# datawhalechina/torch-rechub

Measured on AMD Instinct MI355X. Metric: CTR train samples/sec, DeepFM Criteo-shape synthetic, higher is better.
Workload: dtype f32

## Files before the change

torch_rechub_amd/csrc/optim.hip:

```cpp
#include "common.h"
#include "wgrad_body.h"

namespace {

constexpr int kMaxTensors = 128;
constexpr int kMaxRing = 1024;
int g_sweep_grid = 0;
int g_deferred_grid = 512;
int g_gate_ns = 32000;
int g_stagger_ns = 15000;

constexpr int kVecPerThread = 4;
constexpr int kChunk4 = RH_BLOCK * kVecPerThread;

struct AdamArgs {
  const int64_t* tdesc;
  const double* hyper;
  int T;
  int zero_grad;
  int64_t total_vblocks;
  int64_t vb_prefix[kMaxTensors + 1];
};

__global__ void adam_prepare_kernel(double* hyper, int64_t* step, float* ring, int64_t ring_mask) {
// ... 17 lines not shown
      ring[2 * (t & ring_mask) + 1] = (float)E;
    }
  }
}

struct AdamScalars {
  float b1, b2, wd, one_m_b1, one_m_b2;
  float c1wd, c2wd2;
  float A, E;
};

static __device__ __forceinline__ void adam_elem(float& p, float g, float& m, float& v, const AdamScalars& h, float A,
                                                 float E) {
  g = fmaf(h.wd, p, g);
  m = fmaf(h.one_m_b1, g - m, m);
  v = fmaf(h.one_m_b2, g * g, v * h.b2);
  p = fmaf(-A, m * __builtin_amdgcn_rcpf(__builtin_amdgcn_sqrtf(v) + E), p);
}
typedef float rh_v2f __attribute__((ext_vector_type(2)));
static __device__ __forceinline__ void adam_pair(rh_v2f& p, rh_v2f g, rh_v2f& m, rh_v2f& v, const AdamScalars& h,
                                                 float A, float E) {
  g = __builtin_elementwise_fma(rh_v2f{h.wd, h.wd}, p, g);
  m = __builtin_elementwise_fma(rh_v2f{h.one_m_b1, h.one_m_b1}, g - m, m);
  v = __builtin_elementwise_fma(rh_v2f{h.one_m_b2, h.one_m_b2}, g * g, v * h.b2);
  rh_v2f d = rh_v2f{__builtin_amdgcn_sqrtf(v.x), __builtin_amdgcn_sqrtf(v.y)} + E;
  d = rh_v2f{__builtin_amdgcn_rcpf(d.x), __builtin_amdgcn_rcpf(d.y)};
  p = __builtin_elementwise_fma(rh_v2f{-A, -A}, m * d, p);
}
static __device__ __forceinline__ void adam_pair_zero_g(rh_v2f& p, rh_v2f& m, rh_v2f& v, const AdamScalars& h, float A,
                                                        float E) {
  m = __builtin_elementwise_fma(rh_v2f{h.c1wd, h.c1wd}, p, m * h.b1);
  v = __builtin_elementwise_fma(rh_v2f{h.c2wd2, h.c2wd2}, p * p, v * h.b2);
  rh_v2f d = rh_v2f{__builtin_amdgcn_sqrtf(v.x), __builtin_amdgcn_sqrtf(v.y)} + E;
  d = rh_v2f{__builtin_amdgcn_rcpf(d.x), __builtin_amdgcn_rcpf(d.y)};
  p = __builtin_elementwise_fma(rh_v2f{-A, -A}, m * d, p);
}
static __device__ __forceinline__ void adam_f4_zero_g(float4& P, float4& M, float4& V, const AdamScalars& h, float A,
                                                      float E) {
  rh_v2f p0{P.x, P.y}, p1{P.z, P.w}, m0{M.x, M.y}, m1{M.z, M.w}, v0{V.x, V.y}, v1{V.z, V.w};
  adam_pair_zero_g(p0, m0, v0, h, A, E);
  adam_pair_zero_g(p1, m1, v1, h, A, E);
  P = make_float4(p0.x, p0.y, p1.x, p1.y);
  M = make_float4(m0.x, m0.y, m1.x, m1.y);
  V = make_float4(v0.x, v0.y, v1.x, v1.y);
}
static __device__ __forceinline__ void adam_f4(float4& P, const float4 G, float4& M, float4& V, const AdamScalars& h,
                                               float A, float E) {
  float4 Pz = P, Mz = M, Vz = V;
  adam_f4_zero_g(Pz, Mz, Vz, h, A, E);
  rh_v2f p0{P.x, P.y}, p1{P.z, P.w}, m0{M.x, M.y}, m1{M.z, M.w}, v0{V.x, V.y}, v1{V.z, V.w};
  adam_pair(p0, rh_v2f{G.x, G.y}, m0, v0, h, A, E);
  adam_pair(p1, rh_v2f{G.z, G.w}, m1, v1, h, A, E);
  P = make_float4(G.x == 0.f ? Pz.x : p0.x, G.y == 0.f ? Pz.y : p0.y, G.z == 0.f ? Pz.z : p1.x, G.w == 0.f ? Pz.w : p1.y);
  M = make_float4(G.x == 0.f ? Mz.x : m0.x, G.y == 0.f ? Mz.y : m0.y, G.z == 0.f ? Mz.z : m1.x, G.w == 0.f ? Mz.w : m1.y);
  V = make_float4(G.x == 0.f ? Vz.x : v0.x, G.y == 0.f ? Vz.y : v0.y, G.z == 0.f ? Vz.z : v1.x, G.w == 0.f ? Vz.w : v1.y);
}
static __device__ __forceinline__ AdamScalars load_scalars(const double* hyper) {
  AdamScalars h;
  h.b1 = (float)hyper[1];
  h.b2 = (float)hyper[2];
  h.wd = (float)hyper[4];
  h.one_m_b1 = (float)hyper[10];
  h.one_m_b2 = (float)hyper[11];
  h.c1wd = h.one_m_b1 * h.wd;
  h.c2wd2 = h.one_m_b2 * h.wd * h.wd;
  h.A = (float)hyper[13];
  h.E = (float)hyper[14];
  return h;
}

__global__ __launch_bounds__(RH_BLOCK) void adam_dense_kernel(const AdamArgs a) {
  const AdamScalars h = load_scalars(a.hyper);
  const int T = a.T;
  for (int64_t vb = blockIdx.x; vb < a.total_vblocks; vb += gridDim.x) {
    int lo = 0, hi = T;
    while (hi - lo > 1) {
      const int mid = (lo + hi) >> 1;
      if (a.vb_prefix[mid] <= vb) lo = mid; else hi = mid;
    }
    const int t = lo;
    float* p = reinterpret_cast<float*>(a.tdesc[0 * T + t]);
    float* g = reinterpret_cast<float*>(a.tdesc[1 * T + t]);
    float* m = reinterpret_cast<float*>(a.tdesc[2 * T + t]);
    float* v = reinterpret_cast<float*>(a.tdesc[3 * T + t]);
    const int64_t n4 = a.tdesc[4 * T + t] / 4;
    const int64_t base4 = (vb - a.vb_prefix[t]) * kChunk4;
    float4 P[kVecPerThread], Gv[kVecPerThread], M[kVecPerThread], V[kVecPerThread];
    bool ok[kVecPerThread];
#pragma unroll
    for (int k = 0; k < kVecPerThread; ++k) {
      const int64_t i4 = base4 + (int64_t)k * RH_BLOCK + threadIdx.x;
      ok[k] = i4 < n4;
      const int64_t j4 = ok[k] ? i4 : 0;
      P[k] = gload<float4>(p + j4 * 4);
      Gv[k] = gload<float4>(g + j4 * 4);
      M[k] = gload<float4>(m + j4 * 4);
      V[k] = gload<float4>(v + j4 * 4);
    }
#pragma unroll
    for (int k = 0; k < kVecPerThread; ++k) {
      if (!ok[k]) continue;
      const int64_t i4 = base4 + (int64_t)k * RH_BLOCK + threadIdx.x;
      const bool gnz = Gv[k].x != 0.f || Gv[k].y != 0.f || Gv[k].z != 0.f || Gv[k].w != 0.f;
      adam_f4(P[k], Gv[k], M[k], V[k], h, h.A, h.E);
      gstore<float4>(p + i4 * 4, P[k]);
      gstore<float4>(m + i4 * 4, M[k]);
      gstore<float4>(v + i4 * 4, V[k]);
      if (a.zero_grad && gnz) gstore<float4>(g + i4 * 4, f4_zero());
    }
  }
}


struct LazyTouchedArgs {
  const int64_t* ldesc;
  const int64_t* field_table;
  const int64_t* idesc;
  const double* hyper;
  const float* ring;
  int ring_mask;
  int T, B, F, spb;
  int* err;
  const int64_t* perm;
  const int64_t* pos;
  int64_t N;
  const int64_t* src_sparse;
  int Fd;
  const float* src_dense;
  int ND;
  const float* src_label;
  int64_t* sparse_out;
  float* dense_out;
  float* label_out;
  int look;
  int look_n;
  int64_t off;
};

struct LazySweepArgs {
  const int64_t* ldesc;
  const double* hyper;
  const float* ring;
  int ring_mask;
  int T;
  int flush;
  int64_t t_value;
  int64_t total_vblocks;
  int64_t vb_prefix[kMaxTensors + 1];
  int touch_blocks, touch_chunks, touch_period;
  int touch_i32;
  LazyTouchedArgs touch;
};

template <int LPR, typename IdxT, bool REFRESH, bool ASSEMBLE = false, bool LOOK = false, bool GRAD = !REFRESH>
static __device__ __forceinline__ void lazy_touched_body(const LazyTouchedArgs& a, int bx, int f);

template <int LPR, bool MERGED>
static __device__ __forceinline__ void lazy_sweep_body(const LazySweepArgs& a, const int bx_, const int gdim_) {
  constexpr int RPB = RH_BLOCK / LPR;
  constexpr int D = 4 * LPR;
  int64_t bid = bx_, nblk = gdim_;
  if (MERGED) {
    const int bx = bx_, P = a.touch_period;
    const int slot_ = bx / P;
    if (bx % P == 0 && slot_ < a.touch_blocks) {
      if (a.touch_i32)
        lazy_touched_body<LPR, int, false>(a.touch, slot_ % a.touch_chunks, slot_ / a.touch_chunks);
      else
        lazy_touched_body<LPR, int64_t, false>(a.touch, slot_ % a.touch_chunks, slot_ / a.touch_chunks);
      return;
    }
    bid = bx - (slot_ + 1 < a.touch_blocks ? slot_ + 1 : a.touch_blocks);
    nblk = (int64_t)gdim_ - a.touch_blocks;
  }
  AdamScalars h = load_scalars(a.hyper);
  const int t = a.t_value >= 0 ? (int)a.t_value : (int)a.hyper[12];
  if (a.t_value >= 0) {
    h.A = a.ring[2 * (t & a.ring_mask)];
    h.E = a.ring[2 * (t & a.ring_mask) + 1];
  }
  const int T = a.T;
  const int q = threadIdx.x % LPR;
  const int slot = threadIdx.x / LPR;
  __shared__ float ring_s[2 * kMaxRing];
  for (int i = threadIdx.x; i < 2 * (a.ring_mask + 1); i += RH_BLOCK) ring_s[i] = a.ring[i];
  __syncthreads();

  struct Unit {
    float *p, *g, *m, *v;
    int* last;
    int64_t r;
    int old;
    bool live, with_g, claimed;
    float4 P, M, V, G;
  };
  auto fetch = [&](int64_t vb, Unit& u) {
    u.live = false;
    if (vb >= a.total_vblocks) return;
    int lo = 0, hi = T;
    while (hi - lo > 1) {
      const int mid = (lo + hi) >> 1;
      if (a.vb_prefix[mid] <= vb) lo = mid; else hi = mid;
    }
    const int ti = lo;
    u.p = reinterpret_cast<float*>(a.ldesc[0 * T + ti]);
    u.g = reinterpret_cast<float*>(a.ldesc[1 * T + ti]);
    u.m = reinterpret_cast<float*>(a.ldesc[2 * T + ti]);
    u.v = reinterpret_cast<float*>(a.ldesc[3 * T + ti]);
    u.last = reinterpret_cast<int*>(a.ldesc[4 * T + ti]);
    const int64_t rows = a.ldesc[5 * T + ti];
    const int64_t K = a.ldesc[6 * T + ti];
    const int64_t w = a.flush ? rows : a.ldesc[7 * T + ti];
    const int64_t wstart = a.flush ? 0 : ((int64_t)(t - 1) % K) * w;
    const int64_t local = (vb - a.vb_prefix[ti]) * RPB + slot;
    u.r = wstart + local;
    if (local >= w || u.r >= rows) return;
    u.with_g = (K == 1);
    const bool claim = MERGED && K != 1;
    u.claimed = claim;
    if (claim) {
      u.old = t;
      if (q == 0) u.old = atomicMax(u.last + u.r, t);
      u.with_g = true;
    } else {
      u.old = gload<int>(u.last + u.r);
    }
    u.P = gload<float4>(u.p + u.r * D + q * 4);
    u.M = gload<float4>(u.m + u.r * D + q * 4);
    u.V = gload<float4>(u.v + u.r * D + q * 4);
    u.G = u.with_g ? gload<float4>(u.g + u.r * D + q * 4) : f4_zero();
    if (claim) u.old = __shfl(u.old, (int)(threadIdx.x % RH_WAVE) - q, RH_WAVE);
    u.live = true;
  };
  auto process = [&](Unit& u) {
    const bool work = u.live && u.old < t;
    const int first = work ? u.old + 1 : t;
    int j = wave_min_uniform(first);
    while (j < t) {
      const int nxt = wave_min_uniform(first > j ? first : t);
      if (first <= j) {
        int jj = j;
        for (; jj + 2 <= nxt; jj += 2) {
          const float2 ae0 = *reinterpret_cast<const float2*>(ring_s + 2 * (jj & a.ring_mask));
          const float2 ae1 = *reinterpret_cast<const float2*>(ring_s + 2 * ((jj + 1) & a.ring_mask));
          __builtin_amdgcn_sched_barrier(0);
          adam_f4_zero_g(u.P, u.M, u.V, h, ae0.x, ae0.y);
          adam_f4_zero_g(u.P, u.M, u.V, h, ae1.x, ae1.y);
        }
        if (jj < nxt) {
          const float2 ae = *reinterpret_cast<const float2*>(ring_s + 2 * (jj & a.ring_mask));
          adam_f4_zero_g(u.P, u.M, u.V, h, ae.x, ae.y);
        }
      }
      j = nxt;
    }
    if (work) {
      if (u.with_g) adam_f4(u.P, u.G, u.M, u.V, h, h.A, h.E);
      else adam_f4_zero_g(u.P, u.M, u.V, h, h.A, h.E);
      gstore<float4>(u.p + u.r * D + q * 4, u.P);
      gstore<float4>(u.m + u.r * D + q * 4, u.M);
      gstore<float4>(u.v + u.r * D + q * 4, u.V);
      if (u.with_g && (u.G.x != 0.f || u.G.y != 0.f || u.G.z != 0.f || u.G.w != 0.f))
        gstore<float4>(u.g + u.r * D + q * 4, f4_zero());
      if (q == 0 && !(MERGED && u.with_g && u.claimed)) u.last[u.r] = t;
    }
  };
  Unit ua, ub;
  fetch(bid, ua);
  for (int64_t vb = bid; vb < a.total_vblocks; vb += 2 * nblk) {
    fetch(vb + nblk, ub);
    process(ua);
    fetch(vb + 2 * nblk, ua);
    process(ub);
  }
}

template <int LPR, bool MERGED = false>
__global__ __launch_bounds__(RH_BLOCK) void adam_lazy_sweep_kernel(const LazySweepArgs a) {
  lazy_sweep_body<LPR, MERGED>(a, (int)blockIdx.x, (int)gridDim.x);
}

template <int LPR, int VPL>
static __device__ __forceinline__ void lazy_sweep_wide_body(const LazySweepArgs& a, const int bx_, const int gdim_) {
  constexpr int RPB = RH_BLOCK / LPR;
  constexpr int D = 4 * LPR * VPL;
  const int64_t bid = bx_, nblk = gdim_;
  AdamScalars h = load_scalars(a.hyper);
  const int t = (int)a.t_value;
  h.A = a.ring[2 * (t & a.ring_mask)];
  h.E = a.ring[2 * (t & a.ring_mask) + 1];
  const int T = a.T;
  const int q = threadIdx.x % LPR;
  const int slot = threadIdx.x / LPR;
  __shared__ float ring_s[2 * kMaxRing];
  for (int i = threadIdx.x; i < 2 * (a.ring_mask + 1); i += RH_BLOCK) ring_s[i] = a.ring[i];
  __syncthreads();
  struct Unit {
    float *p, *m, *v;
    int* last;
    int64_t off;
    int64_t r;
    int old;
    bool live;
    float4 P[VPL], M[VPL], V[VPL];
  };
  auto fetch = [&](int64_t vb, Unit& u) {
    u.live = false;
    if (vb >= a.total_vblocks) return;
    int lo = 0, hi = T;
    while (hi - lo > 1) {
      const int mid = (lo + hi) >> 1;
      if (a.vb_prefix[mid] <= vb) lo = mid; else hi = mid;
    }
    const int ti = lo;
    u.p = reinterpret_cast<float*>(a.ldesc[0 * T + ti]);
    u.m = reinterpret_cast<float*>(a.ldesc[2 * T + ti]);
    u.v = reinterpret_cast<float*>(a.ldesc[3 * T + ti]);
    u.last = reinterpret_cast<int*>(a.ldesc[4 * T + ti]);
    const int64_t rows = a.ldesc[5 * T + ti];
    const int64_t K = a.ldesc[6 * T + ti];
    const int64_t w = a.ldesc[7 * T + ti];
    const int64_t wstart = ((int64_t)(t - 1) % K) * w;
    const int64_t local = (vb - a.vb_prefix[ti]) * RPB + slot;
    u.r = wstart + local;
    if (local >= w || u.r >= rows) return;
    u.off = u.r * D + (int64_t)q * (4 * VPL);
    u.old = gload<int>(u.last + u.r);
#pragma unroll
    for (int k = 0; k < VPL; ++k) {
      u.P[k] = gload<float4>(u.p + u.off + 4 * k);
      u.M[k] = gload<float4>(u.m + u.off + 4 * k);
      u.V[k] = gload<float4>(u.v + u.off + 4 * k);
    }
    u.live = true;
  };
  auto process = [&](Unit& u) {
    const bool work = u.live && u.old < t;
    const int first = work ? u.old + 1 : t;
    int j = wave_min_uniform(first);
    while (j < t) {
      const int nxt = wave_min_uniform(first > j ? first : t);
      if (first <= j) {
        int jj = j;
        for (; jj + 2 <= nxt; jj += 2) {
          const float2 ae0 = *reinterpret_cast<const float2*>(ring_s + 2 * (jj & a.ring_mask));
          const float2 ae1 = *reinterpret_cast<const float2*>(ring_s + 2 * ((jj + 1) & a.ring_mask));
          __builtin_amdgcn_sched_barrier(0);
#pragma unroll
          for (int k = 0; k < VPL; ++k) adam_f4_zero_g(u.P[k], u.M[k], u.V[k], h, ae0.x, ae0.y);
#pragma unroll
          for (int k = 0; k < VPL; ++k) adam_f4_zero_g(u.P[k], u.M[k], u.V[k], h, ae1.x, ae1.y);
        }
        if (jj < nxt) {
          const float2 ae = *reinterpret_cast<const float2*>(ring_s + 2 * (jj & a.ring_mask));
#pragma unroll
          for (int k = 0; k < VPL; ++k) adam_f4_zero_g(u.P[k], u.M[k], u.V[k], h, ae.x, ae.y);
        }
      }
      j = nxt;
    }
    if (work) {
#pragma unroll
      for (int k = 0; k < VPL; ++k) {
        adam_f4_zero_g(u.P[k], u.M[k], u.V[k], h, h.A, h.E);
        gstore<float4>(u.p + u.off + 4 * k, u.P[k]);
        gstore<float4>(u.m + u.off + 4 * k, u.M[k]);
        gstore<float4>(u.v + u.off + 4 * k, u.V[k]);
      }
      if (q == 0) u.last[u.r] = t;
    }
  };
  Unit ua, ub;
  fetch(bid, ua);
  for (int64_t vb = bid; vb < a.total_vblocks; vb += 2 * nblk) {
    fetch(vb + nblk, ub);
    process(ua);
    fetch(vb + 2 * nblk, ua);
    process(ub);
  }
}

template <int LPR, int VPL>
__global__ __launch_bounds__(RH_BLOCK) void adam_lazy_sweep_wide_kernel(const LazySweepArgs a) {
  lazy_sweep_wide_body<LPR, VPL>(a, (int)blockIdx.x, (int)gridDim.x);
}

__global__ void stream_delay_kernel(const long long ticks) {
  const long long t0 = wall_clock64();
  while (wall_clock64() - t0 < ticks) __builtin_amdgcn_s_sleep(16);
}

__global__ void stream_gate_kernel(const long long* gate, const long long expected, const long long ticks, const long long timeout,
                                   int* err, long long* done_host, const long long done_value) {
  if (done_host != nullptr) __hip_atomic_store(done_host, done_value, __ATOMIC_RELAXED, __HIP_MEMORY_SCOPE_SYSTEM);
  const long long t0 = wall_clock64();
  while (__hip_atomic_load(gate, __ATOMIC_ACQUIRE, __HIP_MEMORY_SCOPE_AGENT) - expected < 0) {
    __builtin_amdgcn_s_sleep(8);
    if (wall_clock64() - t0 > timeout) {
      if (err != nullptr) atomicOr(err, RH_ERR_GATE_TIMEOUT);
      return;
    }
  }
  const int slot = 4 + 2 * (int)(expected & 3);
  const long long base = __hip_atomic_load(gate + slot, __ATOMIC_RELAXED, __HIP_MEMORY_SCOPE_AGENT);
  const long long opened = __hip_atomic_load(gate + slot + 1, __ATOMIC_RELAXED, __HIP_MEMORY_SCOPE_AGENT);
  while (__hip_atomic_load(gate + 2, __ATOMIC_RELAXED, __HIP_MEMORY_SCOPE_AGENT) - base < 1 && wall_clock64() - opened < ticks)
    __builtin_amdgcn_s_sleep(4);
}

static __device__ __forceinline__ void gate_open(long long* gate) {
  const long long idx = __hip_atomic_load(gate, __ATOMIC_RELAXED, __HIP_MEMORY_SCOPE_AGENT) + 1;
  const int slot = 4 + 2 * (int)(idx & 3);
  const long long now = (long long)wall_clock64();
  __hip_atomic_store(gate + slot, __hip_atomic_load(gate + 2, __ATOMIC_RELAXED, __HIP_MEMORY_SCOPE_AGENT), __ATOMIC_RELAXED,
                     __HIP_MEMORY_SCOPE_AGENT);
  __hip_atomic_store(gate + slot + 1, now, __ATOMIC_RELAXED, __HIP_MEMORY_SCOPE_AGENT);
  __hip_atomic_store(gate + 1, now, __ATOMIC_RELAXED, __HIP_MEMORY_SCOPE_AGENT);
  __hip_atomic_fetch_add(gate, 1ll, __ATOMIC_RELEASE, __HIP_MEMORY_SCOPE_AGENT);
}

__global__ void stream_gate_open_kernel(long long* gate) { gate_open(gate); }
__global__ void stream_gate_release_kernel(long long* gate) {
  __hip_atomic_fetch_add(gate + 2, 1ll, __ATOMIC_RELAXED, __HIP_MEMORY_SCOPE_AGENT);
}

template <int LPR, typename IdxT, bool REFRESH, bool ASSEMBLE, bool LOOK, bool GRAD>
static __device__ __forceinline__ void lazy_touched_body(const LazyTouchedArgs& a, int bx, int f) {
  constexpr int LPP = RH_BLOCK / LPR;
  constexpr int D = 4 * LPR;
  const int T = a.T, F = a.F;
  const int64_t ti = a.field_table[f];
  if (ti < 0) return;
  const int64_t K = a.ldesc[6 * T + ti];
  if (K == 1) return;
  const int64_t pad = a.field_table[F + f];
  float* p = reinterpret_cast<float*>(a.ldesc[0 * T + ti]);
  float* g = reinterpret_cast<float*>(a.ldesc[1 * T + ti]);
  float* m = reinterpret_cast<float*>(a.ldesc[2 * T + ti]);
  float* v = reinterpret_cast<float*>(a.ldesc[3 * T + ti]);
  int* last = reinterpret_cast<int*>(a.ldesc[4 * T + ti]);
  const int64_t rows = a.ldesc[5 * T + ti];
  const IdxT* ip = reinterpret_cast<const IdxT*>(a.idesc[f]);
  const int64_t st = a.idesc[F + f];
  const int64_t acol = ASSEMBLE ? (reinterpret_cast<const int64_t*>(ip) - a.sparse_out) : 0;
  const int64_t apos = ASSEMBLE ? a.pos[0] : 0;
  const AdamScalars h = load_scalars(a.hyper);
  const int t = (int)a.hyper[12];
  const int q = threadIdx.x % LPR;
  const int slot = threadIdx.x / LPR;
  const int lane = threadIdx.x % RH_WAVE;
  const int64_t nsamp = LOOK ? a.look_n : a.B;
  int64_t b0 = (int64_t)bx * (LOOK ? a.look : a.spb);
  int64_t b1 = (b0 + (LOOK ? a.look : a.spb) < nsamp) ? b0 + (LOOK ? a.look : a.spb) : nsamp;
  __shared__ float ring_t[REFRESH ? 2 * kMaxRing : 2];
  if (REFRESH) {
    for (int i = threadIdx.x; i < 2 * (a.ring_mask + 1); i += RH_BLOCK) ring_t[i] = a.ring[i];
    __syncthreads();
  }
  const float* ring = REFRESH ? ring_t : a.ring;
  const bool pad_pass = !LOOK && REFRESH && pad >= 0 && pad < rows && bx == 0;
  __shared__ int64_t s_look[LOOK ? RH_BLOCK : 1];
  __shared__ int s_nlook;
  const int64_t look_b1 = b1;
  for (int64_t sub = LOOK ? b0 : 0; sub < (LOOK ? look_b1 : 1); sub += RH_BLOCK) {
  if (LOOK) {
    const int64_t w = a.ldesc[7 * T + ti];
    const int64_t ws = ((int64_t)(t - 1) % K) * w;
    if (threadIdx.x == 0) s_nlook = 0;
    __syncthreads();
    const int64_t b = sub + threadIdx.x;
    if (b < look_b1) {
      const int64_t p = (apos + a.off + (int64_t)a.B + b) % a.N;
      const int64_t r = gload<int64_t>(a.src_sparse + gload<int64_t>(a.perm + p) * a.Fd + acol);
      if (r >= ws && r < ws + w && r < rows && r != pad) s_look[atomicAdd(&s_nlook, 1)] = r;
    }
    __syncthreads();
    b0 = 0;
    b1 = s_nlook;
  }
  const int64_t b_end = b1 + (pad_pass ? LPP : 0);
  for (int64_t base = b0; base < b_end; base += LPP) {
    const bool extra = base >= b1;
    const int64_t b = base + slot;
    const bool ok = !extra && b < b1;
    int64_t r;
    if (LOOK) {
      r = s_look[ok ? b : 0];
    } else if (ASSEMBLE) {
      int64_t p = apos + a.off + (ok ? b : b1 - 1);
      if (p >= a.N) p %= a.N;
      if (p < 0) p += a.N;
      r = gload<int64_t>(a.src_sparse + gload<int64_t>(a.perm + p) * a.Fd + acol);
    } else {
      r = (int64_t)gload<IdxT>(ip + (ok ? b : b1 - 1) * st);
    }
    bool valid = ok && (uint64_t)r < (uint64_t)rows && r != pad;
    if (extra) {
      r = pad;
      valid = slot == 0;
    }
    int old = t;
    if (valid && q == 0) {
      old = gload<int>(last + r);
      if (old < t) old = atomicMax(last + r, t);
    }
    old = __shfl(old, lane - q, RH_WAVE);
    bool act = valid && old < t;
    int64_t rr = r;
    if (REFRESH) {
      __shared__ int s_key[LPP];
      __shared__ int s_old[LPP];
      __shared__ int64_t s_row[LPP];
      const int lag = act ? t - old : 0;
      __syncthreads();
      if (q == 0) s_key[slot] = lag;
      __syncthreads();
      int rank = 0;
#pragma unroll 4
      for (int j = 0; j < LPP; ++j) {
        const int kj = s_key[j];
        rank += (kj > lag || (kj == lag && j < slot)) ? 1 : 0;
      }
      constexpr int kPerWave = RH_WAVE / LPR;
      rank = (rank + (bx % (LPP / kPerWave > 0 ? LPP / kPerWave : 1)) * kPerWave) % LPP;
      if (q == 0) {
        s_row[rank] = r;
        s_old[rank] = act ? old : t;
      }
      __syncthreads();
      rr = s_row[slot];
      old = s_old[slot];
      act = old < t;
    }
    float4 P = f4_zero(), M = f4_zero(), V = f4_zero(), G = f4_zero();
    if (act) {
      P = gload<float4>(p + rr * D + q * 4);
      M = gload<float4>(m + rr * D + q * 4);
      V = gload<float4>(v + rr * D + q * 4);
      if (GRAD) G = gload<float4>(g + rr * D + q * 4);
    }
    const int first = act ? old + 1 : t;
    int j = wave_min_uniform(first);
    while (j < t) {
      const int nxt = wave_min_uniform(first > j ? first : t);
      if (first <= j) {
        for (int jj = j; jj < nxt; ++jj) {
          const float A = ring[2 * (jj & a.ring_mask)], E = ring[2 * (jj & a.ring_mask) + 1];
          adam_f4_zero_g(P, M, V, h, A, E);
        }
      }
      j = nxt;
    }
    if (!act) continue;
    if (GRAD) adam_f4(P, G, M, V, h, h.A, h.E);
    else adam_f4_zero_g(P, M, V, h, h.A, h.E);
    gstore<float4>(p + rr * D + q * 4, P);
    gstore<float4>(m + rr * D + q * 4, M);
    gstore<float4>(v + rr * D + q * 4, V);
    if (GRAD && (!REFRESH || G.x != 0.f || G.y != 0.f || G.z != 0.f || G.w != 0.f)) gstore<float4>(g + rr * D + q * 4, f4_zero());
  }
  }
}

template <int LPR, typename IdxT, bool REFRESH>
__global__ __launch_bounds__(RH_BLOCK) void adam_lazy_touched_kernel(const LazyTouchedArgs a) {
  RH_CHAIN_PRIO();
  lazy_touched_body<LPR, IdxT, REFRESH>(a, (int)blockIdx.x, (int)blockIdx.y);
}

constexpr int kTouchGroup = 4;
struct LazyTouchedGroupArgs {
  LazyTouchedArgs rec[kTouchGroup];
  int prefix[kTouchGroup + 1];
  int chunks[kTouchGroup];
  int i64[kTouchGroup];
  int n;
};

template <int LPR, bool REFRESH>
__global__ __launch_bounds__(RH_BLOCK) void adam_lazy_touched_group_kernel(const LazyTouchedGroupArgs g) {
  RH_CHAIN_PRIO();
  const int bx = (int)blockIdx.x;
  int i = 0;
#pragma unroll
  for (int k = 1; k < kTouchGroup; ++k) i += (k < g.n && bx >= g.prefix[k]) ? 1 : 0;
  const int local = bx - g.prefix[i];
#pragma unroll
  for (int k = 0; k < kTouchGroup; ++k) {
    if (k == i) {
      if (g.i64[k]) lazy_touched_body<LPR, int64_t, REFRESH>(g.rec[k], local % g.chunks[k], local / g.chunks[k]);
      else lazy_touched_body<LPR, int, REFRESH>(g.rec[k], local % g.chunks[k], local / g.chunks[k]);
      return;
    }
  }
}

template <int LPR>
__global__ __launch_bounds__(RH_BLOCK) void adam_lazy_refresh_assemble_kernel(const LazyTouchedArgs a) {
  RH_CHAIN_PRIO();
  if ((int)blockIdx.y < a.F) {
    lazy_touched_body<LPR, int64_t, true, true>(a, (int)blockIdx.x, (int)blockIdx.y);
    return;
  }
  if ((int)blockIdx.y > a.F) {
    const int R = a.look / a.spb;
    const int f = ((int)blockIdx.y - a.F - 1) * R + (int)blockIdx.x % R;
    if (f < a.F) lazy_touched_body<LPR, int64_t, true, true, true>(a, (int)blockIdx.x / R, f);
    return;
  }
  constexpr int G = 16;
  const int lig = threadIdx.x % G;
  const int64_t pos = a.pos[0];
  const int64_t b0 = (int64_t)blockIdx.x * a.spb;
  const int64_t b1 = (b0 + a.spb < (int64_t)a.B) ? b0 + a.spb : (int64_t)a.B;
  for (int64_t b = b0 + threadIdx.x / G; b < b1; b += RH_BLOCK / G) {
    int64_t p = pos + b;
    if (p >= a.N) p %= a.N;
    const int64_t src = a.perm[p];
    for (int j = lig; j < a.Fd; j += G) a.sparse_out[b * a.Fd + j] = a.src_sparse[src * a.Fd + j];
    for (int j = lig; j < a.ND; j += G) a.dense_out[b * a.ND + j] = a.src_dense[src * a.ND + j];
    if (lig == 0 && a.src_label != nullptr) a.label_out[b] = a.src_label[src];
  }
}

struct StepAheadParts {
  int nB, chunksB;
  int spbB;
  int nA, chunksA;
  int spbA;
  int nC, chunksC;
  int nD;
  const int64_t* idescA;
  int BA;
};

template <int LPR>
__device__ __forceinline__ void step_ahead_body(const LazySweepArgs& a, const StepAheadParts& parts, int bx, const int nblocks) {
  if (bx < parts.nB) {
    LazyTouchedArgs ta = a.touch;
    ta.spb = parts.spbB;
    ta.off = 0;
    lazy_touched_body<LPR, int64_t, true, true, false, true>(ta, bx % parts.chunksB, bx / parts.chunksB);
    return;
  }
  bx -= parts.nB;
  if (bx < parts.nA) {
    LazyTouchedArgs ta = a.touch;
    ta.spb = parts.spbA;
    if (parts.BA > 0) {
      ta.idesc = parts.idescA;
      ta.B = parts.BA;
      ta.off = 0;
      lazy_touched_body<LPR, int64_t, false, false, false, true>(ta, bx % parts.chunksA, bx / parts.chunksA);
      return;
    }
    ta.off = -(int64_t)ta.B;
    lazy_touched_body<LPR, int64_t, false, true, false, true>(ta, bx % parts.chunksA, bx / parts.chunksA);
    return;
  }
  bx -= parts.nA;
  if (bx < parts.nC) {
    LazyTouchedArgs ta = a.touch;
    ta.off = 0;
    lazy_touched_body<LPR, int64_t, true, true, true, true>(ta, bx % parts.chunksC, bx / parts.chunksC);
    return;
  }
  bx -= parts.nC;
  if (bx < parts.nD) {
    const LazyTouchedArgs& ta = a.touch;
    constexpr int G = 16;
    const int lig = threadIdx.x % G;
    const int64_t pos = ta.pos[0];
    const int64_t b0 = (int64_t)bx * parts.spbB;
    const int64_t b1 = (b0 + parts.spbB < (int64_t)ta.B) ? b0 + parts.spbB : (int64_t)ta.B;
    for (int64_t b = b0 + threadIdx.x / G; b < b1; b += RH_BLOCK / G) {
      int64_t p = pos + b;
      if (p >= ta.N) p %= ta.N;
      const int64_t src = ta.perm[p];
      for (int j = lig; j < ta.Fd; j += G) ta.sparse_out[b * ta.Fd + j] = ta.src_sparse[src * ta.Fd + j];
      for (int j = lig; j < ta.ND; j += G) ta.dense_out[b * ta.ND + j] = ta.src_dense[src * ta.ND + j];
      if (lig == 0 && ta.src_label != nullptr) ta.label_out[b] = ta.src_label[src];
    }
    return;
  }
  bx -= parts.nD;
  lazy_sweep_body<LPR, true>(a, bx, nblocks - parts.nB - parts.nA - parts.nC - parts.nD);
}

template <int LPR>
__global__ __launch_bounds__(RH_BLOCK) void adam_lazy_step_ahead_kernel(const LazySweepArgs a, const StepAheadParts parts) {
  RH_CHAIN_PRIO();
  step_ahead_body<LPR>(a, parts, (int)blockIdx.x, (int)gridDim.x);
}

template <int LPR>
__global__ __launch_bounds__(RH_BLOCK) __attribute__((amdgpu_waves_per_eu(4, 4))) void adam_lazy_step_ahead_wgrad_kernel(
    const LazySweepArgs a, const StepAheadParts parts, const rh_wgrad::WgradGroupArgs ga) {
  RH_CHAIN_PRIO();
  extern __shared__ float wred[];
  const int nW = ga.prefix[rh_wgrad::kWgradGroup];
  const int nrest = (int)gridDim.x - nW;
  const int bx = (int)blockIdx.x;
  if (bx >= nrest) {
    rh_wgrad::linear_wgrad_group_body<true>(ga, wred, bx - nrest);
    return;
  }
  step_ahead_body<LPR>(a, parts, bx, nrest);
}

template <int LPR, int VPL>
int launch_sweep_wide(LazySweepArgs& a, const int64_t* h_rows, const int64_t* h_window, hipStream_t s) {
  constexpr int RPB = RH_BLOCK / LPR;
  a.vb_prefix[0] = 0;
  for (int t = 0; t < a.T; ++t) {
    int64_t w = h_window[t] < h_rows[t] ? h_window[t] : h_rows[t];
    if (h_window[t] >= h_rows[t]) w = 0;
    a.vb_prefix[t + 1] = a.vb_prefix[t] + (w + RPB - 1) / RPB;
  }
  for (int t = a.T + 1; t <= kMaxTensors; ++t) a.vb_prefix[t] = a.vb_prefix[a.T];
  a.total_vblocks = a.vb_prefix[a.T];
  a.touch_blocks = a.touch_chunks = 0;
  a.touch_period = 1;
  if (a.total_vblocks == 0) return 0;
  int64_t grid = a.total_vblocks;
  const int64_t cap = g_deferred_grid > 0 ? g_deferred_grid : (g_sweep_grid > 0 ? g_sweep_grid : 256 * 32);
  if (grid > cap) grid = cap;
  hipLaunchKernelGGL((adam_lazy_sweep_wide_kernel<LPR, VPL>), dim3((unsigned)grid), dim3(RH_BLOCK), 0, s, a);
  return 0;
}

template <int LPR>
int launch_sweep(LazySweepArgs& a, int mode, const int64_t* h_rows, const int64_t* h_window, hipStream_t s,
                 const LazyTouchedArgs* touch = nullptr) {
  constexpr int RPB = RH_BLOCK / LPR;
  if constexpr (LPR >= 2) {
    if (mode == RH_SWEEP_LAZY_TABLES && a.t_value >= 0 && touch == nullptr)
      return launch_sweep_wide<LPR / 2, 2>(a, h_rows, h_window, s);
  }
  a.vb_prefix[0] = 0;
  for (int t = 0; t < a.T; ++t) {
    int64_t w = a.flush ? h_rows[t] : (h_window[t] < h_rows[t] ? h_window[t] : h_rows[t]);
    const bool dense_table = h_window[t] >= h_rows[t];
    if ((mode == RH_SWEEP_LAZY_TABLES && dense_table) || (mode == RH_SWEEP_DENSE_TABLES && !dense_table)) w = 0;
    a.vb_prefix[t + 1] = a.vb_prefix[t] + (w + RPB - 1) / RPB;
  }
  for (int t = a.T + 1; t <= kMaxTensors; ++t) a.vb_prefix[t] = a.vb_prefix[a.T];
  a.total_vblocks = a.vb_prefix[a.T];
  a.touch_blocks = a.touch_chunks = 0;
  a.touch_period = 1;
  if (touch != nullptr) {
    a.touch = *touch;
    a.touch_chunks = (touch->B + touch->spb - 1) / touch->spb;
    a.touch_blocks = a.touch_chunks * touch->F;
  }
  if (a.total_vblocks == 0 && a.touch_blocks == 0) return 0;
  int64_t grid = a.total_vblocks;
  const int64_t cap = (a.t_value >= 0 && touch == nullptr && g_deferred_grid > 0) ? g_deferred_grid
                      : (g_sweep_grid > 0 ? g_sweep_grid : 256 * 32);
  if (grid > cap) grid = cap;
  if (touch != nullptr) {
    if (grid < 1) grid = 1;
    int64_t period = (grid + a.touch_blocks) / a.touch_blocks;
    if (period > 1 && period % 8 == 0) period -= 1;
    a.touch_period = (int)period;
    hipLaunchKernelGGL((adam_lazy_sweep_kernel<LPR, true>), dim3((unsigned)(grid + a.touch_blocks)), dim3(RH_BLOCK), 0, s,
                       a);
  } else {
    hipLaunchKernelGGL((adam_lazy_sweep_kernel<LPR, false>), dim3((unsigned)grid), dim3(RH_BLOCK), 0, s, a);
  }
  return 0;
}


struct AdamSmallArgs {
  const int64_t* sdesc;
  const float* flat_g;
  const double* hyper;
  int T;
  int64_t total_vblocks;
  int64_t vb_prefix[kMaxTensors + 1];
};
constexpr int kSmallChunk = 1024;

__global__ __launch_bounds__(RH_BLOCK) void adam_small_kernel(const AdamSmallArgs a) {
  RH_CHAIN_PRIO();
  const AdamScalars h = load_scalars(a.hyper);
  const int T = a.T;
  for (int64_t vb = blockIdx.x; vb < a.total_vblocks; vb += gridDim.x) {
    int lo = 0, hi = T;
    while (hi - lo > 1) {
      const int mid = (lo + hi) >> 1;
      if (a.vb_prefix[mid] <= vb) lo = mid; else hi = mid;
    }
    const int t = lo;
    float* p = reinterpret_cast<float*>(a.sdesc[0 * T + t]);
    float* m = reinterpret_cast<float*>(a.sdesc[1 * T + t]);
    float* v = reinterpret_cast<float*>(a.sdesc[2 * T + t]);
    const int64_t n = a.sdesc[3 * T + t];
    const float* g = a.flat_g + a.sdesc[4 * T + t];
    const int64_t base = (vb - a.vb_prefix[t]) * kSmallChunk;
#pragma unroll
    for (int k = 0; k < kSmallChunk / RH_BLOCK; ++k) {
      const int64_t i = base + (int64_t)k * RH_BLOCK + threadIdx.x;
      if (i < n) {
        float P = p[i], M = m[i], V = v[i];
        adam_elem(P, g[i], M, V, h, h.A, h.E);
        p[i] = P;
        m[i] = M;
        v[i] = V;
      }
    }
  }
}

constexpr int kPackItems = 32;
struct PackArgs {
  RhPackItem it[kPackItems];
  int64_t vb_prefix[kPackItems + 1];
  int n;
  float* flat;
// ... 396 lines not shown
  return 0;
}

extern "C" int rh_adam_lazy_refresh_assemble(const int64_t* ldesc, int T, const int64_t* field_table, const int64_t* idesc, int B,
                                             int F, int D, const double* hyper, const float* ring, int ring_size,
                                             int samples_per_block, int32_t* err_flag, const int64_t* perm, const int64_t* pos,
                                             int64_t N, const int64_t* sparse, int Fd, const float* dense, int ND,
                                             const float* label, int64_t* sparse_out, float* dense_out, float* label_out,
                                             int lookahead, void* stream) {
  RH_REQUIRE(ldesc && field_table && idesc && hyper && ring && perm && pos && sparse && sparse_out, RH_E_BADARG,
             "rh_adam_lazy_refresh_assemble: null pointer");
  RH_REQUIRE(T >= 1 && F >= 1 && F <= 65534 && B >= 1 && N >= 1 && Fd >= 1 && ND >= 0, RH_E_BADARG,
             "rh_adam_lazy_refresh_assemble: bad shape");
  RH_REQUIRE(ND == 0 || (dense && dense_out), RH_E_BADARG, "rh_adam_lazy_refresh_assemble: dense pointers null");
  RH_REQUIRE(label == nullptr || label_out != nullptr, RH_E_BADARG, "rh_adam_lazy_refresh_assemble: label_out null");
  RH_REQUIRE(ring_size > 0 && (ring_size & (ring_size - 1)) == 0 && ring_size <= kMaxRing, RH_E_BADARG,
             "rh_adam_lazy_refresh_assemble: ring_size must be a power of two <= %d", kMaxRing);
  const int spb = samples_per_block <= 0 ? 64 : ((samples_per_block + 63) / 64) * 64;
  const int chunks = (B + spb - 1) / spb;
  int R = RH_BLOCK / spb >= 1 ? RH_BLOCK / spb : 1;
  if (chunks % R != 0) R = 1;
  LazyTouchedArgs a{ldesc, field_table, idesc, hyper, ring, ring_size - 1, T, B, F, spb, err_flag,
                    perm, pos, N, sparse, Fd, dense, ND, label, sparse_out, dense_out, label_out, lookahead ? R * spb : 0,
                    lookahead ? B : 0, 0};
  const dim3 grid((unsigned)chunks, (unsigned)(F + 1 + (lookahead ? (F + R - 1) / R : 0)));
  hipStream_t s = reinterpret_cast<hipStream_t>(stream);
  switch (D / 4) {
    case 1: hipLaunchKernelGGL((adam_lazy_refresh_assemble_kernel<1>), grid, dim3(RH_BLOCK), 0, s, a); break;
    case 2: hipLaunchKernelGGL((adam_lazy_refresh_assemble_kernel<2>), grid, dim3(RH_BLOCK), 0, s, a); break;
    case 4: hipLaunchKernelGGL((adam_lazy_refresh_assemble_kernel<4>), grid, dim3(RH_BLOCK), 0, s, a); break;
    case 8: hipLaunchKernelGGL((adam_lazy_refresh_assemble_kernel<8>), grid, dim3(RH_BLOCK), 0, s, a); break;
    case 16: hipLaunchKernelGGL((adam_lazy_refresh_assemble_kernel<16>), grid, dim3(RH_BLOCK), 0, s, a); break;
    case 32: hipLaunchKernelGGL((adam_lazy_refresh_assemble_kernel<32>), grid, dim3(RH_BLOCK), 0, s, a); break;
    default: rh_set_error("rh_adam_lazy_refresh_assemble: embed_dim %d unsupported", D); return RH_E_UNSUPPORTED;
  }
  RH_LAUNCH_CHECK("rh_adam_lazy_refresh_assemble");
  return 0;
}

static int lazy_step_impl(const int64_t* ldesc, int T, const int64_t* h_rows, const int64_t* h_window, int D,
                          const double* hyper, const float* ring, int ring_size, const int64_t* field_table,
                          const int64_t* idesc, int B, int F, int samples_per_block, int32_t* err_flag, int sweep_mode,
                          int idx_is_i64, void* stream) {
  RH_REQUIRE(ldesc && h_rows && h_window && hyper && ring && field_table && idesc, RH_E_BADARG,
             "rh_adam_lazy_step: null pointer");
  RH_REQUIRE(T >= 1 && T <= kMaxTensors && F >= 1 && F <= 65535 && B >= 1, RH_E_BADARG, "rh_adam_lazy_step: bad shape");
  RH_REQUIRE(ring_size > 0 && (ring_size & (ring_size - 1)) == 0 && ring_size <= kMaxRing, RH_E_BADARG,
             "rh_adam_lazy_step: ring_size must be a power of two <= %d", kMaxRing);
  const int spb = samples_per_block <= 0 ? 256 : ((samples_per_block + 63) / 64) * 64;
  LazyTouchedArgs ta{ldesc, field_table, idesc, hyper, ring, ring_size - 1, T, B, F, spb, err_flag};
  LazySweepArgs a{};
  a.ldesc = ldesc;
  a.hyper = hyper;
  a.ring = ring;
  a.ring_mask = ring_size - 1;
  a.T = T;
  a.flush = 0;
  a.t_value = -1;
  a.touch_i32 = idx_is_i64 ? 0 : 1;
  hipStream_t s = reinterpret_cast<hipStream_t>(stream);
  int rc = RH_E_UNSUPPORTED;
  switch (D / 4) {
    case 1: rc = launch_sweep<1>(a, sweep_mode, h_rows, h_window, s, &ta); break;
    case 2: rc = launch_sweep<2>(a, sweep_mode, h_rows, h_window, s, &ta); break;
    case 4: rc = launch_sweep<4>(a, sweep_mode, h_rows, h_window, s, &ta); break;
    case 8: rc = launch_sweep<8>(a, sweep_mode, h_rows, h_window, s, &ta); break;
    case 16: rc = launch_sweep<16>(a, sweep_mode, h_rows, h_window, s, &ta); break;
    case 32: rc = launch_sweep<32>(a, sweep_mode, h_rows, h_window, s, &ta); break;
    default: break;
  }
  RH_REQUIRE(rc == 0 && D % 4 == 0, RH_E_UNSUPPORTED, "rh_adam_lazy_step: embed_dim %d unsupported", D);
  RH_LAUNCH_CHECK("rh_adam_lazy_step");
  return 0;
}

static int step_ahead_impl(const int64_t* ldesc, int T, const int64_t* h_rows, const int64_t* h_window, int D,
                           const double* hyper, const float* ring, int ring_size, const int64_t* field_table,
                           const int64_t* idesc, int B, int F, int32_t* err_flag, const int64_t* perm, const int64_t* pos,
                           int64_t N, const int64_t* sparse, int Fd, const float* dense, int ND, const float* label,
                           int64_t* sparse_out, float* dense_out, float* label_out, int look_depth,
                           const rh_wgrad::WgradGroupArgs* ga, const int64_t* touched_idesc, int touched_B, void* stream);

extern "C" int rh_adam_lazy_step_ahead(const int64_t* ldesc, int T, const int64_t* h_rows, const int64_t* h_window, int D,
                                       const double* hyper, const float* ring, int ring_size, const int64_t* field_table,
                                       const int64_t* idesc, int B, int F, int32_t* err_flag, const int64_t* perm,
                                       const int64_t* pos, int64_t N, const int64_t* sparse, int Fd, const float* dense, int ND,
                                       const float* label, int64_t* sparse_out, float* dense_out, float* label_out,
                                       int look_depth, void* stream) {
  return step_ahead_impl(ldesc, T, h_rows, h_window, D, hyper, ring, ring_size, field_table, idesc, B, F, err_flag, perm, pos, N,
                         sparse, Fd, dense, ND, label, sparse_out, dense_out, label_out, look_depth, nullptr, nullptr, 0, stream);
}

extern "C" int rh_adam_lazy_step_ahead_touched(const int64_t* ldesc, int T, const int64_t* h_rows, const int64_t* h_window, int D,
                                               const double* hyper, const float* ring, int ring_size,
                                               const int64_t* field_table, const int64_t* idesc, int B, int F, int32_t* err_flag,
                                               const int64_t* perm, const int64_t* pos, int64_t N, const int64_t* sparse, int Fd,
                                               const float* dense, int ND, const float* label, int64_t* sparse_out,
                                               float* dense_out, float* label_out, int look_depth,
                                               const int64_t* touched_idesc, int touched_B, void* stream) {
  RH_REQUIRE(touched_idesc != nullptr && touched_B >= 1, RH_E_BADARG, "rh_adam_lazy_step_ahead_touched: no touched index matrix");
  return step_ahead_impl(ldesc, T, h_rows, h_window, D, hyper, ring, ring_size, field_table, idesc, B, F, err_flag, perm, pos, N,
                         sparse, Fd, dense, ND, label, sparse_out, dense_out, label_out, look_depth, nullptr, touched_idesc,
                         touched_B, stream);
}

extern "C" int rh_adam_lazy_step_ahead_wgrad(const int64_t* ldesc, int T, const int64_t* h_rows, const int64_t* h_window, int D,
                                             const double* hyper, const float* ring, int ring_size, const int64_t* field_table,
                                             const int64_t* idesc, int B, int F, int32_t* err_flag, const int64_t* perm,
                                             const int64_t* pos, int64_t N, const int64_t* sparse, int Fd, const float* dense,
                                             int ND, const float* label, int64_t* sparse_out, float* dense_out, float* label_out,
                                             int look_depth, int wn, const float* const* wg, const int64_t* wldg,
                                             const float* const* wx, const int64_t* wldx, const int* wB, const int* wN,
                                             const int* wK, float* const* wpartial, void* stream) {
  rh_wgrad::WgradGroupArgs ga;
  const int rc = rh_wgrad_group_fill(wn, wg, wldg, wx, wldx, wB, wN, wK, wpartial, &ga, "rh_adam_lazy_step_ahead_wgrad");
  if (rc != 0) return rc;
  return step_ahead_impl(ldesc, T, h_rows, h_window, D, hyper, ring, ring_size, field_table, idesc, B, F, err_flag, perm, pos, N,
                         sparse, Fd, dense, ND, label, sparse_out, dense_out, label_out, look_depth, &ga, nullptr, 0, stream);
}

static int step_ahead_impl(const int64_t* ldesc, int T, const int64_t* h_rows, const int64_t* h_window, int D,
                           const double* hyper, const float* ring, int ring_size, const int64_t* field_table,
                           const int64_t* idesc, int B, int F, int32_t* err_flag, const int64_t* perm, const int64_t* pos,
                           int64_t N, const int64_t* sparse, int Fd, const float* dense, int ND, const float* label,
                           int64_t* sparse_out, float* dense_out, float* label_out, int look_depth,
                           const rh_wgrad::WgradGroupArgs* ga, const int64_t* touched_idesc, int touched_B, void* stream) {
  RH_REQUIRE(ldesc && h_rows && h_window && hyper && ring && field_table && idesc && perm && pos && sparse && sparse_out,
             RH_E_BADARG, "rh_adam_lazy_step_ahead: null pointer");
  RH_REQUIRE(T >= 1 && T <= kMaxTensors && F >= 1 && F <= 65535 && B >= 1 && N >= B && Fd >= 1 && ND >= 0 && look_depth >= 0 &&
                 look_depth <= 4, RH_E_BADARG, "rh_adam_lazy_step_ahead: bad shape");
  RH_REQUIRE(ND == 0 || (dense && dense_out), RH_E_BADARG, "rh_adam_lazy_step_ahead: dense pointers null");
  RH_REQUIRE(label == nullptr || label_out != nullptr, RH_E_BADARG, "rh_adam_lazy_step_ahead: label_out null");
  RH_REQUIRE(ring_size > 0 && (ring_size & (ring_size - 1)) == 0 && ring_size <= kMaxRing, RH_E_BADARG,
             "rh_adam_lazy_step_ahead: ring_size must be a power of two <= %d", kMaxRing);
  LazySweepArgs a{};
  a.ldesc = ldesc;
  a.hyper = hyper;
  a.ring = ring;
  a.ring_mask = ring_size - 1;
  a.T = T;
  a.flush = 0;
  a.t_value = -1;
  a.vb_prefix[0] = 0;
  for (int t = 0; t < T; ++t) {
    const bool dense_table = h_window[t] >= h_rows[t];
    const int64_t w = dense_table ? h_rows[t] : 0;
    const int rpb = RH_BLOCK / (D / 4);
    a.vb_prefix[t + 1] = a.vb_prefix[t] + (w + rpb - 1) / rpb;
  }
  for (int t = T + 1; t <= kMaxTensors; ++t) a.vb_prefix[t] = a.vb_prefix[T];
  a.total_vblocks = a.vb_prefix[T];
  a.touch_blocks = a.touch_chunks = 0;
  a.touch_period = 1;
  const int look = RH_BLOCK;
  a.touch = LazyTouchedArgs{ldesc, field_table, idesc, hyper, ring, ring_size - 1, T, B, F, 64, err_flag,
                            perm, pos, N, sparse, Fd, dense, ND, label, sparse_out, dense_out, label_out,
                            look, look_depth * B, 0};
  StepAheadParts parts;
  parts.spbB = 64;
  parts.chunksB = (B + parts.spbB - 1) / parts.spbB;
  parts.nB = parts.chunksB * F;
  parts.spbA = 256;
  parts.idescA = touched_idesc;
  parts.BA = touched_idesc != nullptr ? touched_B : 0;
  parts.chunksA = ((parts.BA > 0 ? parts.BA : B) + parts.spbA - 1) / parts.spbA;
  parts.nA = parts.chunksA * F;
  parts.chunksC = (look_depth * B + look - 1) / look;
  parts.nC = parts.chunksC * F;
  parts.nD = parts.chunksB;
  int64_t sweep_grid = a.total_vblocks;
  const int64_t cap = g_sweep_grid > 0 ? g_sweep_grid : 256 * 32;
  if (sweep_grid > cap) sweep_grid = cap;
  if (sweep_grid < 1) sweep_grid = 1;
  hipStream_t s = reinterpret_cast<hipStream_t>(stream);
  if (ga != nullptr) {
    const dim3 gridw((unsigned)(ga->prefix[rh_wgrad::kWgradGroup] + parts.nB + parts.nA + parts.nC + parts.nD + sweep_grid));
    const size_t lds = (size_t)rh_wgrad::kPartStride * sizeof(float);
    switch (D / 4) {
      case 1: hipLaunchKernelGGL((adam_lazy_step_ahead_wgrad_kernel<1>), gridw, dim3(RH_BLOCK), lds, s, a, parts, *ga); break;
      case 2: hipLaunchKernelGGL((adam_lazy_step_ahead_wgrad_kernel<2>), gridw, dim3(RH_BLOCK), lds, s, a, parts, *ga); break;
      case 4: hipLaunchKernelGGL((adam_lazy_step_ahead_wgrad_kernel<4>), gridw, dim3(RH_BLOCK), lds, s, a, parts, *ga); break;
      case 8: hipLaunchKernelGGL((adam_lazy_step_ahead_wgrad_kernel<8>), gridw, dim3(RH_BLOCK), lds, s, a, parts, *ga); break;
      case 16: hipLaunchKernelGGL((adam_lazy_step_ahead_wgrad_kernel<16>), gridw, dim3(RH_BLOCK), lds, s, a, parts, *ga); break;
      case 32: hipLaunchKernelGGL((adam_lazy_step_ahead_wgrad_kernel<32>), gridw, dim3(RH_BLOCK), lds, s, a, parts, *ga); break;
      default: rh_set_error("rh_adam_lazy_step_ahead_wgrad: embed_dim %d unsupported", D); return RH_E_UNSUPPORTED;
    }
    RH_LAUNCH_CHECK("rh_adam_lazy_step_ahead_wgrad");
    return 0;
  }
  const dim3 grid((unsigned)(parts.nB + parts.nA + parts.nC + parts.nD + sweep_grid));
  switch (D / 4) {
    case 1: hipLaunchKernelGGL((adam_lazy_step_ahead_kernel<1>), grid, dim3(RH_BLOCK), 0, s, a, parts); break;
    case 2: hipLaunchKernelGGL((adam_lazy_step_ahead_kernel<2>), grid, dim3(RH_BLOCK), 0, s, a, parts); break;
    case 4: hipLaunchKernelGGL((adam_lazy_step_ahead_kernel<4>), grid, dim3(RH_BLOCK), 0, s, a, parts); break;
    case 8: hipLaunchKernelGGL((adam_lazy_step_ahead_kernel<8>), grid, dim3(RH_BLOCK), 0, s, a, parts); break;
    case 16: hipLaunchKernelGGL((adam_lazy_step_ahead_kernel<16>), grid, dim3(RH_BLOCK), 0, s, a, parts); break;
    case 32: hipLaunchKernelGGL((adam_lazy_step_ahead_kernel<32>), grid, dim3(RH_BLOCK), 0, s, a, parts); break;
    default: rh_set_error("rh_adam_lazy_step_ahead: embed_dim %d unsupported", D); return RH_E_UNSUPPORTED;
  }
  RH_LAUNCH_CHECK("rh_adam_lazy_step_ahead");
  return 0;
}

extern "C" int rh_adam_small(const int64_t* sdesc, int T, const int64_t* h_numel, const float* flat_g,
                             const double* hyper, void* stream) {
  RH_REQUIRE(sdesc && h_numel && flat_g && hyper, RH_E_BADARG, "rh_adam_small: null pointer");
  RH_REQUIRE(T >= 1 && T <= kMaxTensors, RH_E_UNSUPPORTED, "rh_adam_small: T=%d (max %d tensors per call)", T,
             kMaxTensors);
  AdamSmallArgs a;
  a.sdesc = sdesc;
  a.flat_g = flat_g;
  a.hyper = hyper;
  a.T = T;
  a.vb_prefix[0] = 0;
  for (int t = 0; t < T; ++t) {
    RH_REQUIRE(h_numel[t] >= 0, RH_E_BADARG, "rh_adam_small: negative numel");
    a.vb_prefix[t + 1] = a.vb_prefix[t] + (h_numel[t] + kSmallChunk - 1) / kSmallChunk;
  }
  for (int t = T + 1; t <= kMaxTensors; ++t) a.vb_prefix[t] = a.vb_prefix[T];
  a.total_vblocks = a.vb_prefix[T];
  if (a.total_vblocks == 0) return 0;
  int64_t grid = a.total_vblocks;
  if (grid > 256 * 16) grid = 256 * 16;
  hipLaunchKernelGGL(adam_small_kernel, dim3((unsigned)grid), dim3(RH_BLOCK), 0, reinterpret_cast<hipStream_t>(stream),
                     a);
  RH_LAUNCH_CHECK("rh_adam_small");
  return 0;
}

extern "C" int rh_adam_lazy_step(const int64_t* ldesc, int T, const int64_t* h_rows, const int64_t* h_window, int D,
                                 const double* hyper, const float* ring, int ring_size, const int64_t* field_table,
                                 const int64_t* idesc, int B, int F, int samples_per_block, int32_t* err_flag,
                                 void* stream) {
  return lazy_step_impl(ldesc, T, h_rows, h_window, D, hyper, ring, ring_size, field_table, idesc, B, F, samples_per_block,
                        err_flag, RH_SWEEP_WINDOW, 1, stream);
}

extern "C" int rh_adam_lazy_step_mode(const int64_t* ldesc, int T, const int64_t* h_rows, const int64_t* h_window, int D,
                                      const double* hyper, const float* ring, int ring_size, const int64_t* field_table,
                                      const int64_t* idesc, int B, int F, int samples_per_block, int32_t* err_flag,
                                      int sweep_mode, void* stream) {
  RH_REQUIRE(sweep_mode == RH_SWEEP_WINDOW || sweep_mode == RH_SWEEP_DENSE_TABLES, RH_E_BADARG,
             "rh_adam_lazy_step_mode: sweep_mode %d", sweep_mode);
  return lazy_step_impl(ldesc, T, h_rows, h_window, D, hyper, ring, ring_size, field_table, idesc, B, F, samples_per_block,
                        err_flag, sweep_mode, 1, stream);
}

extern "C" int rh_adam_lazy_step_mode_idx(const int64_t* ldesc, int T, const int64_t* h_rows, const int64_t* h_window, int D,
                                          const double* hyper, const float* ring, int ring_size, const int64_t* field_table,
                                          const int64_t* idesc, int idx_is_i64, int B, int F, int samples_per_block,
                                          int32_t* err_flag, int sweep_mode, void* stream) {
  RH_REQUIRE(sweep_mode == RH_SWEEP_WINDOW || sweep_mode == RH_SWEEP_DENSE_TABLES, RH_E_BADARG,
             "rh_adam_lazy_step_mode_idx: sweep_mode %d", sweep_mode);
  return lazy_step_impl(ldesc, T, h_rows, h_window, D, hyper, ring, ring_size, field_table, idesc, B, F, samples_per_block,
                        err_flag, sweep_mode, idx_is_i64, stream);
}
```

Baseline: 18.62 million.

## Batch lookahead row scans across rounds and schedule lookahead blocks first

The lookahead phase of the step-ahead kernel now gathers candidate rows over several rounds of RH_BLOCK samples per block, with the index loads issued together, and accumulates matches in a larger shared buffer before processing. Each block covers 2*4*RH_BLOCK samples, so fewer blocks are launched and fewer process passes run per scanned row. The lookahead blocks move to the front of the grid so this longer work starts early. The ring buffer in shared memory becomes a single shared allocation across the sweep and touched bodies to cut LDS usage. The larger s_look array raises shared memory per block, and fewer lookahead blocks may reduce parallelism.

Measured after the change: 18.87 million (median of 6 runs). +1.3%, better.

```diff
diff --git a/torch_rechub_amd/csrc/optim.hip b/torch_rechub_amd/csrc/optim.hip
--- a/torch_rechub_amd/csrc/optim.hip
+++ b/torch_rechub_amd/csrc/optim.hip
@@ -193,8 +193,14 @@
   LazyTouchedArgs touch;
 };
 
-template <int LPR, typename IdxT, bool REFRESH, bool ASSEMBLE = false, bool LOOK = false, bool GRAD = !REFRESH>
+template <int LPR, typename IdxT, bool REFRESH, bool ASSEMBLE = false, bool LOOK = false, bool GRAD = !REFRESH,
+          int LOOKR = 1>
 static __device__ __forceinline__ void lazy_touched_body(const LazyTouchedArgs& a, int bx, int f);
+
+static __device__ __forceinline__ float* ring_lds() {
+  __shared__ float ring_shared[2 * kMaxRing];
+  return ring_shared;
+}
 
 template <int LPR, bool MERGED>
 static __device__ __forceinline__ void lazy_sweep_body(const LazySweepArgs& a, const int bx_, const int gdim_) {
@@ -223,7 +229,7 @@
   const int T = a.T;
   const int q = threadIdx.x % LPR;
   const int slot = threadIdx.x / LPR;
-  __shared__ float ring_s[2 * kMaxRing];
+  float* const ring_s = ring_lds();
   for (int i = threadIdx.x; i < 2 * (a.ring_mask + 1); i += RH_BLOCK) ring_s[i] = a.ring[i];
   __syncthreads();
 
@@ -465,7 +471,7 @@
   __hip_atomic_fetch_add(gate + 2, 1ll, __ATOMIC_RELAXED, __HIP_MEMORY_SCOPE_AGENT);
 }
 
-template <int LPR, typename IdxT, bool REFRESH, bool ASSEMBLE, bool LOOK, bool GRAD>
+template <int LPR, typename IdxT, bool REFRESH, bool ASSEMBLE, bool LOOK, bool GRAD, int LOOKR>
 static __device__ __forceinline__ void lazy_touched_body(const LazyTouchedArgs& a, int bx, int f) {
   constexpr int LPP = RH_BLOCK / LPR;
   constexpr int D = 4 * LPR;
@@ -493,31 +499,48 @@
   const int64_t nsamp = LOOK ? a.look_n : a.B;
   int64_t b0 = (int64_t)bx * (LOOK ? a.look : a.spb);
   int64_t b1 = (b0 + (LOOK ? a.look : a.spb) < nsamp) ? b0 + (LOOK ? a.look : a.spb) : nsamp;
-  __shared__ float ring_t[REFRESH ? 2 * kMaxRing : 2];
+  float* const ring_t = REFRESH ? ring_lds() : nullptr;
   if (REFRESH) {
     for (int i = threadIdx.x; i < 2 * (a.ring_mask + 1); i += RH_BLOCK) ring_t[i] = a.ring[i];
     __syncthreads();
   }
   const float* ring = REFRESH ? ring_t : a.ring;
   const bool pad_pass = !LOOK && REFRESH && pad >= 0 && pad < rows && bx == 0;
-  __shared__ int64_t s_look[LOOK ? RH_BLOCK : 1];
+  constexpr int kLookRounds = LOOKR;
+  constexpr int kLookCap = (kLookRounds + 1) * RH_BLOCK;
+  constexpr int kLookFlush = RH_BLOCK;
+  static_assert(kLookFlush + kLookRounds * RH_BLOCK <= kLookCap, "s_look: carried rows + one round's rows must fit");
+  __shared__ int64_t s_look[LOOK ? kLookCap : 1];
   __shared__ int s_nlook;
   const int64_t look_b1 = b1;
-  for (int64_t sub = LOOK ? b0 : 0; sub < (LOOK ? look_b1 : 1); sub += RH_BLOCK) {
+  bool look_fresh = true;
+  for (int64_t sub = LOOK ? b0 : 0; sub < (LOOK ? look_b1 : 1); sub += kLookRounds * RH_BLOCK) {
   if (LOOK) {
     const int64_t w = a.ldesc[7 * T + ti];
     const int64_t ws = ((int64_t)(t - 1) % K) * w;
-    if (threadIdx.x == 0) s_nlook = 0;
+    if (look_fresh && threadIdx.x == 0) s_nlook = 0;
     __syncthreads();
-    const int64_t b = sub + threadIdx.x;
-    if (b < look_b1) {
-      const int64_t p = (apos + a.off + (int64_t)a.B + b) % a.N;
-      const int64_t r = gload<int64_t>(a.src_sparse + gload<int64_t>(a.perm + p) * a.Fd + acol);
+    int64_t rl[kLookRounds];
+#pragma unroll
+    for (int u = 0; u < kLookRounds; ++u) {
+      const int64_t b = sub + (int64_t)u * RH_BLOCK + threadIdx.x;
+      rl[u] = -1;
+      if (b < look_b1) {
+        const int64_t p = (apos + a.off + (int64_t)a.B + b) % a.N;
+        rl[u] = gload<int64_t>(a.src_sparse + gload<int64_t>(a.perm + p) * a.Fd + acol);
+      }
+    }
+#pragma unroll
+    for (int u = 0; u < kLookRounds; ++u) {
+      const int64_t r = rl[u];
       if (r >= ws && r < ws + w && r < rows && r != pad) s_look[atomicAdd(&s_nlook, 1)] = r;
     }
     __syncthreads();
+    const int n = s_nlook;
+    look_fresh = sub + kLookRounds * RH_BLOCK >= look_b1 || n > kLookFlush;
+    if (!look_fresh) continue;
     b0 = 0;
-    b1 = s_nlook;
+    b1 = n;
   }
   const int64_t b_end = b1 + (pad_pass ? LPP : 0);
   for (int64_t base = b0; base < b_end; base += LPP) {
@@ -664,6 +687,9 @@
   }
 }
 
+constexpr int kAheadLookRounds = 4;
+constexpr int kAheadLookSamples = 2 * kAheadLookRounds * RH_BLOCK;
+
 struct StepAheadParts {
   int nB, chunksB;
   int spbB;
@@ -677,6 +703,13 @@
 
 template <int LPR>
 __device__ __forceinline__ void step_ahead_body(const LazySweepArgs& a, const StepAheadParts& parts, int bx, const int nblocks) {
+  if (bx < parts.nC) {
+    LazyTouchedArgs ta = a.touch;
+    ta.off = 0;
+    lazy_touched_body<LPR, int64_t, true, true, true, true, kAheadLookRounds>(ta, bx % parts.chunksC, bx / parts.chunksC);
+    return;
+  }
+  bx -= parts.nC;
   if (bx < parts.nB) {
     LazyTouchedArgs ta = a.touch;
     ta.spb = parts.spbB;
@@ -700,13 +733,6 @@
     return;
   }
   bx -= parts.nA;
-  if (bx < parts.nC) {
-    LazyTouchedArgs ta = a.touch;
-    ta.off = 0;
-    lazy_touched_body<LPR, int64_t, true, true, true, true>(ta, bx % parts.chunksC, bx / parts.chunksC);
-    return;
-  }
-  bx -= parts.nC;
   if (bx < parts.nD) {
     const LazyTouchedArgs& ta = a.touch;
     constexpr int G = 16;
@@ -1409,7 +1435,7 @@
   a.total_vblocks = a.vb_prefix[T];
   a.touch_blocks = a.touch_chunks = 0;
   a.touch_period = 1;
-  const int look = RH_BLOCK;
+  const int look = kAheadLookSamples;
   a.touch = LazyTouchedArgs{ldesc, field_table, idesc, hyper, ring, ring_size - 1, T, B, F, 64, err_flag,
                             perm, pos, N, sparse, Fd, dense, ND, label, sparse_out, dense_out, label_out,
                             look, look_depth * B, 0};
```
